# GreptimeTeam/greptimedb

Hardware: AMD Instinct MI355X
Metric: TSBS DevOps ingest rows/sec (whole node) (higher is better)
Workload: dtype f64; 1 GPU; model=tsbs-devops-cpu-only, global_batch=3000, seq_len=0, parallelism=region-shard dp1, scale_per_worker=100, workers=6, pool_rows=2394000, rows_shipped_cross_rank=0, wal=group-commit, no fsync, flush_mb=64, ssts_written=6, device=cuda:0

## Files before the change

csrc/ingest_core.h:

```cpp

#pragma once

#include <cmath>
#include <cstdint>
#include <cstdlib>
#include <cstring>
#include <limits>
#include <string>
#include <utility>
#include <vector>

namespace gdb_ingest {


static inline uint64_t load64(const char* p) {
  uint64_t v;
  std::memcpy(&v, p, 8);
  return v;
}

static inline uint64_t mix64(uint64_t a, uint64_t b) {
  const __uint128_t r = (__uint128_t)a * b;
  return (uint64_t)r ^ (uint64_t)(r >> 64);
}

static inline uint64_t hash64(const char* p, size_t n) {
  const uint64_t K0 = 0x9E3779B97F4A7C15ULL, K1 = 0xA0761D6478BD642FULL,
                 K2 = 0xE7037ED1A0B428DBULL;
  const char* const end = p + n;
  uint64_t s0 = K0 ^ n, s1 = K2;
  size_t left = n;
  while (left >= 32) {
    s0 = mix64(load64(p) ^ K1, load64(p + 8) ^ s0);
// ... 245 lines not shown
  std::vector<std::string> field_names_;
  std::vector<std::pair<size_t, size_t>> fcache_;
  std::vector<uint64_t> stamp_;
  uint64_t stamp_ctr_ = 0;
};


static inline size_t align8(size_t x) { return (x + 7) & ~(size_t)7; }

struct StageLayout {
  size_t ts, fields, dst_off, series, region, total;
  StageLayout(size_t n, size_t nf) {
    ts = 0;
    fields = 8 * n;
    dst_off = fields + 8 * nf * n;
    series = dst_off + 8 * n;
    region = series + align8(4 * n);
    total = region + align8(4 * n);
  }
};

constexpr int kMaxPackedRegions = 16;

enum FusedStatus { FUSED_OK = 0, FUSED_SLOW = 1, FUSED_GROW = 2 };

struct FusedResult {
  FusedStatus status = FUSED_SLOW;
  size_t n = 0;
  size_t need_bytes = 0;
  std::vector<int64_t> counts, mins, maxs;
  std::vector<char> wal;
  std::vector<size_t> wal_off;
  ParseSink sink;
  std::vector<int32_t> own_series;
  std::vector<int64_t> own_ts;
  std::vector<double> own_cols;
};

static inline void fused_ingest(
    LineCore& core, const char* buf, size_t len,
    const int32_t* sid_region, const int32_t* sid_local, size_t lut_len,
    const int64_t* fmap, int nf, size_t n_parser_fields, int n_regions,
    const std::string& hdr_suffix, bool durable, int64_t ts_scale,
    char* stage, size_t stage_bytes, FusedResult& out) {
  const size_t est = LineCore::count_lines(buf, len);
  const size_t F = core.num_fields();
  bool direct = lut_len > 0 && n_regions > 0 && n_regions <= kMaxPackedRegions &&
                n_parser_fields == F && est > 0;
  if (direct) {
    for (int t = 0; t < nf; t++)
      if (fmap[t] >= (int64_t)F) direct = false;
  }
  if (direct) {
    const StageLayout need(est, (size_t)nf);
    if (need.total > stage_bytes) {
      out.status = FUSED_GROW;
      out.need_bytes = need.total;
      return;
    }
  }
  ParseSink& sink = out.sink;
  sink.cap = est;
  sink.col.assign(F, nullptr);
  const StageLayout L(est, (size_t)nf);
  if (direct) {
    sink.ts = reinterpret_cast<int64_t*>(stage + L.ts);
    sink.series = reinterpret_cast<int32_t*>(stage + L.series);
// ... 59 lines not shown
    const int32_t r = sid_region[sid];
    series[i] = sid_local[sid];
    region[i] = r;
    dst_off[i] = cnt[r]++;
    const int64_t t_ns = (int64_t)((uint64_t)ts[i] * (uint64_t)ts_scale);
    int64_t t = t_ns / 1000000;
    if (t_ns % 1000000 < 0) t--;
    ts[i] = t;
    if (t < mn[r]) mn[r] = t;
    if (t > mx[r]) mx[r] = t;
  }
  out.status = FUSED_OK;
  out.wal_off.assign((size_t)n_regions + 1, 0);
  if (!durable) return;

  std::vector<std::string> hdrs(n_regions);
  std::vector<size_t> code_off(n_regions), ts_off(n_regions), f_off(n_regions);
  size_t total = 0;
  for (int r = 0; r < n_regions; r++) {
    out.wal_off[r] = total;
    const size_t m = (size_t)cnt[r];
    if (m == 0) continue;
    hdrs[r] = "{\"n\": " + std::to_string(cnt[r]) + hdr_suffix;
    code_off[r] = total + 4 + hdrs[r].size();
    ts_off[r] = code_off[r] + 4 * m;
    f_off[r] = ts_off[r] + 8 * m;
    total = f_off[r] + 8 * (size_t)nf * m;
  }
  out.wal_off[n_regions] = total;
  out.wal.resize(total);
  char* w = out.wal.data();
  for (int r = 0; r < n_regions; r++) {
    if (cnt[r] == 0) continue;
    const uint32_t hl = (uint32_t)hdrs[r].size();
    std::memcpy(w + out.wal_off[r], &hl, 4);
    std::memcpy(w + out.wal_off[r] + 4, hdrs[r].data(), hl);
  }
  for (size_t i = 0; i < n; i++) {
    const int32_t r = region[i];
    const size_t o = (size_t)dst_off[i];
    const size_t m = (size_t)cnt[r];
    std::memcpy(w + code_off[r] + 4 * o, series + i, 4);
    std::memcpy(w + ts_off[r] + 8 * o, ts + i, 8);
    char* fdst = w + f_off[r];
    for (int t = 0; t < nf; t++)
      std::memcpy(fdst + 8 * ((size_t)t * m + o), fields + (size_t)t * n + i, 8);
  }
}

}
```

csrc/ingest_core_check.cpp:

```cpp

#include <cstdio>
#include <random>
#include <string>
#include <vector>

#include "ingest_core.h"

using namespace gdb_ingest;

static int failures = 0;
#define CHECK(cond)                                                    \
  do {                                                                 \
    if (!(cond)) {                                                     \
      std::printf("CHECK failed %s:%d: %s\n", __FILE__, __LINE__, #cond); \
      failures++;                                                      \
    }                                                                  \
  } while (0)

struct Plain {
  std::vector<int32_t> series;
  std::vector<int64_t> ts;
  std::vector<double> cols;
  ParseSink sink;
  size_t n = 0, cap = 0;
// ... 139 lines not shown
    const int64_t* ts = reinterpret_cast<const int64_t*>(stage.data() + L.ts);
    const double* f = reinterpret_cast<const double*>(stage.data() + L.fields);
    const int64_t* dst = reinterpret_cast<const int64_t*>(stage.data() + L.dst_off);
    const int32_t* se = reinterpret_cast<const int32_t*>(stage.data() + L.series);
    const int32_t* rg = reinterpret_cast<const int32_t*>(stage.data() + L.region);
    std::vector<int64_t> cnt(R, 0);
    for (size_t i = 0; i < n; i++) {
      const int32_t sid = p.series[i];
      CHECK(rg[i] == sid % R && se[i] == sid / R);
      CHECK(dst[i] == cnt[rg[i]]);
      cnt[rg[i]]++;
      CHECK(ts[i] == floor_ms(p.ts[i], scale));
      for (int t = 0; t < nf; t++) {
        const double want = fmap[t] < 0 ? std::nan("") : p.sink.col[fmap[t]][i];
        CHECK(same_double(f[(size_t)t * n + i], want));
      }
    }
    size_t wal = 0;
    for (int r = 0; r < R; r++) {
      CHECK(res.counts[r] == cnt[r]);
      const size_t len = res.wal_off[r + 1] - res.wal_off[r];
      if (cnt[r] == 0) { CHECK(len == 0); continue; }
      uint32_t hl;
      std::memcpy(&hl, res.wal.data() + res.wal_off[r], 4);
      CHECK(len == 4 + hl + (size_t)cnt[r] * (12 + 8 * nf));
      wal += len;
    }
    CHECK(wal == res.wal.size());
  }

  {
    FusedResult res;
    const std::string d = "cpu,hostname=brand_new usage_user=1 5\n";
    fused_ingest(core, d.data(), d.size(), sid_region.data(), sid_local.data(),
                 sid_region.size(), fmap.data(), nf, 4, R, suffix, true, 1,
                 stage.data(), stage.size(), res);
    CHECK(res.status == FUSED_SLOW && res.n == 1 && res.sink.new_tagsets.size() == 1);
    CHECK(res.sink.col[0][0] == 1.0 && std::isnan(res.sink.col[1][0]));
  }
  {
    FusedResult res;
    const std::string d = "cpu,hostname=host_1,region=eu-1,rack=7 usage_user=1,fresh=2 5\n";
    fused_ingest(core, d.data(), d.size(), sid_region.data(), sid_local.data(),
                 sid_region.size(), fmap.data(), nf, 4, R, suffix, true, 1,
                 stage.data(), stage.size(), res);
    CHECK(res.status == FUSED_SLOW && res.n == 1 && core.num_fields() == 5);
    CHECK(res.sink.col.size() == 5 && res.sink.col[4][0] == 2.0);
  }
// ... 27 lines not shown
```

csrc/native.cpp:

```cpp

#include <pybind11/pybind11.h>
#include <pybind11/numpy.h>
#include <pybind11/stl.h>

#include <cerrno>
#include <cmath>
#include <cstdint>
#include <cstring>
#include <fcntl.h>
#include <stdexcept>
#include <string>
#include <unistd.h>
#include <unordered_map>
#include <vector>

#include "ingest_core.h"

namespace py = pybind11;

static uint32_t crc_table[8][256];
static bool crc_init_done = [] {
  for (uint32_t i = 0; i < 256; i++) {
    uint32_t c = i;
    for (int k = 0; k < 8; k++) c = (c & 1) ? 0xEDB88320u ^ (c >> 1) : c >> 1;
    crc_table[0][i] = c;
  }
  for (int t = 1; t < 8; t++)
    for (uint32_t i = 0; i < 256; i++)
      crc_table[t][i] = crc_table[0][crc_table[t - 1][i] & 0xFF] ^
                        (crc_table[t - 1][i] >> 8);
  return true;
}();

static uint32_t crc32_update(uint32_t crc, const uint8_t* buf, size_t len) {
  crc = ~crc;
  while (len >= 8) {
    uint32_t lo, hi;
    std::memcpy(&lo, buf, 4);
    std::memcpy(&hi, buf + 4, 4);
    lo ^= crc;
    crc = crc_table[7][lo & 0xFF] ^ crc_table[6][(lo >> 8) & 0xFF] ^
          crc_table[5][(lo >> 16) & 0xFF] ^ crc_table[4][lo >> 24] ^
          crc_table[3][hi & 0xFF] ^ crc_table[2][(hi >> 8) & 0xFF] ^
          crc_table[1][(hi >> 16) & 0xFF] ^ crc_table[0][hi >> 24];
    buf += 8;
    len -= 8;
  }
  for (size_t i = 0; i < len; i++)
    crc = crc_table[0][(crc ^ buf[i]) & 0xFF] ^ (crc >> 8);
  return ~crc;
}

static inline uint64_t fnv1a(const char* p, size_t n) {
  uint64_t h = 1469598103934665603ULL;
  for (size_t i = 0; i < n; i++) { h ^= (uint8_t)p[i]; h *= 1099511628211ULL; }
  return h;
}


static py::capsule owner_of(void* p) {
  return py::capsule(p, [](void* q) { std::free(q); });
}

class LineParser {
 public:
  py::tuple parse(py::bytes data) {
    char* buf;
    Py_ssize_t len;
    if (PyBytes_AsStringAndSize(data.ptr(), &buf, &len) != 0)
      throw std::runtime_error("expected bytes");
    gdb_ingest::ParseSink sink;
    const size_t F0 = core_.num_fields();
    size_t nrows = 0, est = 0;
    int32_t* series = nullptr;
// ... 7 lines not shown
      block = static_cast<double*>(std::malloc(8 * est * F0 + 8));
      if (series && ts && block) {
        sink.series = series;
        sink.ts = ts;
        sink.cap = est;
        sink.col.resize(F0);
        for (size_t c = 0; c < F0; c++) sink.col[c] = block + c * est;
        nrows = core_.parse(buf, (size_t)len, sink);
      }
    }
    py::capsule so = owner_of(series), to = owner_of(ts), bo = owner_of(block);
    if (!series || !ts || !block) throw std::bad_alloc();
    return make_parse_tuple(
        py::array_t<int32_t>({(py::ssize_t)nrows}, {4}, series, so),
        py::array_t<int64_t>({(py::ssize_t)nrows}, {8}, ts, to),
        sink, nrows, F0, bo);
  }

  py::tuple ingest_batch(
      py::bytes data, py::array_t<int32_t, py::array::c_style> sid_region,
      py::array_t<int32_t, py::array::c_style> sid_local,
      py::array_t<int64_t, py::array::c_style> fmap, size_t n_parser_fields,
      int n_regions, py::bytes hdr_suffix, bool durable, int64_t ts_scale,
      py::array_t<uint8_t, py::array::c_style> stage) {
    char* buf;
    Py_ssize_t len;
    if (PyBytes_AsStringAndSize(data.ptr(), &buf, &len) != 0)
      throw std::runtime_error("expected bytes");
    if (sid_region.ndim() != 1 || sid_local.ndim() != 1 || fmap.ndim() != 1 ||
        stage.ndim() != 1 || sid_local.shape(0) != sid_region.shape(0))
      throw std::runtime_error("ingest_batch: bad argument shapes");
    char* sp = reinterpret_cast<char*>(stage.mutable_data());
    if (reinterpret_cast<uintptr_t>(sp) % 8 != 0)
      throw std::runtime_error("ingest_batch: stage must be 8-byte aligned");
    const std::string suffix = hdr_suffix;
    const size_t F0 = core_.num_fields();
    auto* res = new gdb_ingest::FusedResult();
    py::capsule keep(res, [](void* q) {
      delete static_cast<gdb_ingest::FusedResult*>(q);
    });
    {
      py::gil_scoped_release rel;
      gdb_ingest::fused_ingest(
          core_, buf, (size_t)len, sid_region.data(), sid_local.data(),
          (size_t)sid_region.shape(0), fmap.data(), (int)fmap.shape(0),
          n_parser_fields, n_regions, suffix, durable, ts_scale, sp,
          (size_t)stage.shape(0), *res);
    }
    if (res->status == gdb_ingest::FUSED_GROW)
      return py::make_tuple(2, res->need_bytes);
    if (res->status == gdb_ingest::FUSED_SLOW) {
      const size_t n = res->n;
      py::array_t<int32_t> series((py::ssize_t)n);
      py::array_t<int64_t> ts((py::ssize_t)n);
      if (n) {
        std::memcpy(series.mutable_data(), res->sink.series, 4 * n);
        std::memcpy(ts.mutable_data(), res->sink.ts, 8 * n);
      }
      double* block = static_cast<double*>(std::malloc(8 * n * F0 + 8));
      py::capsule bo = owner_of(block);
      if (!block) throw std::bad_alloc();
      for (size_t c = 0; c < F0 && n; c++)
        std::memcpy(block + c * n, res->sink.col[c], 8 * n);
      for (size_t c = 0; c < F0; c++) res->sink.col[c] = block + c * n;
      return py::make_tuple(1, make_parse_tuple(
          std::move(series), std::move(ts), res->sink, n, F0, bo));
    }
    py::array_t<int64_t> counts(n_regions), mins(n_regions), maxs(n_regions);
    py::list payloads;
    if (res->n) {
      std::memcpy(counts.mutable_data(), res->counts.data(), 8 * (size_t)n_regions);
      std::memcpy(mins.mutable_data(), res->mins.data(), 8 * (size_t)n_regions);
      std::memcpy(maxs.mutable_data(), res->maxs.data(), 8 * (size_t)n_regions);
      for (int r = 0; r < n_regions; r++) {
        const size_t lo = res->wal_off[r], hi = res->wal_off[r + 1];
        if (hi == lo) {
          payloads.append(py::none());
        } else {
          payloads.append(py::array_t<uint8_t>(
              {(py::ssize_t)(hi - lo)}, {1},
              reinterpret_cast<const uint8_t*>(res->wal.data() + lo), keep));
        }
      }
    }
    return py::make_tuple(0, res->n, std::move(counts), std::move(mins),
                          std::move(maxs), std::move(payloads));
  }

  size_t num_series() const { return core_.num_series(); }
  std::vector<std::string> field_names() const { return core_.field_names(); }
  size_t num_fields() const { return core_.num_fields(); }
  size_t intern_capacity() const { return core_.intern_capacity(); }

  py::bytes tagset_str(int32_t sid) const {
    const std::string* s = core_.tagset_str(sid);
    if (!s) throw std::out_of_range("unknown series ref");
    return py::bytes(*s);
  }

  void register_tagset(const std::string& s, int32_t id) { core_.register_tagset(s, id); }
  void register_field(const std::string& name) { core_.register_field(name); }

 private:
  py::tuple make_parse_tuple(py::array_t<int32_t> series, py::array_t<int64_t> ts,
// ... 45 lines not shown
  void close_segment() {
    if (fd_ >= 0) { ::close(fd_); fd_ = -1; }
  }

  void append(uint64_t region_id, uint64_t seq, py::object payload) {
    char* pbuf; Py_ssize_t plen;
    Py_buffer view;
    bool have_view = false;
    if (PyBytes_Check(payload.ptr())) {
      if (PyBytes_AsStringAndSize(payload.ptr(), &pbuf, &plen) != 0)
        throw std::runtime_error("payload must be bytes");
    } else {
      if (PyObject_GetBuffer(payload.ptr(), &view, PyBUF_SIMPLE) != 0)
        throw py::error_already_set();
      have_view = true;
      pbuf = static_cast<char*>(view.buf);
      plen = view.len;
    }
    struct Release {
      Py_buffer* v;
      ~Release() { if (v) PyBuffer_Release(v); }
    } release{have_view ? &view : nullptr};
    py::gil_scoped_release rel;
    uint32_t body_len = 16 + static_cast<uint32_t>(plen);
    size_t off = buf_.size();
    buf_.resize(off + 8 + body_len);
    uint8_t* w = buf_.data() + off;
    std::memcpy(w, &body_len, 4);
    uint8_t hdr[16];
    std::memcpy(hdr, &region_id, 8);
    std::memcpy(hdr + 8, &seq, 8);
    uint32_t crc = crc32_update(0, hdr, 16);
    crc = crc32_update(crc, reinterpret_cast<uint8_t*>(pbuf), plen);
    std::memcpy(w + 4, &crc, 4);
    std::memcpy(w + 8, hdr, 16);
    std::memcpy(w + 24, pbuf, plen);
  }

  uint64_t commit(bool sync) {
    if (fd_ < 0) throw std::runtime_error("wal: no open segment");
    size_t n = buf_.size();
    if (n) {
      py::gil_scoped_release rel;
      const uint8_t* p = buf_.data();
      size_t left = n;
      while (left) {
        ssize_t w = ::write(fd_, p, left);
        if (w < 0) {
          if (errno == EINTR) continue;
          throw std::runtime_error(std::string("wal write failed: ") + strerror(errno));
        }
        p += w; left -= w;
      }
      if (sync && ::fdatasync(fd_) != 0)
        throw std::runtime_error(std::string("wal fdatasync failed: ") + strerror(errno));
    }
    buf_.clear();
    seg_bytes_ += n;
    return seg_bytes_;
  }

  uint64_t segment_bytes() const { return seg_bytes_; }

 private:
  int fd_ = -1;
  std::string path_;
  uint64_t seg_bytes_ = 0;
  std::vector<uint8_t> buf_;
};

static py::list wal_read_segment(const std::string& path) {
  py::list out;
  int fd = ::open(path.c_str(), O_RDONLY);
  if (fd < 0) throw std::runtime_error("wal open failed: " + path);
  off_t sz = ::lseek(fd, 0, SEEK_END);
  ::lseek(fd, 0, SEEK_SET);
  std::vector<uint8_t> data(sz);
  size_t got = 0;
  while (got < static_cast<size_t>(sz)) {
    ssize_t r = ::read(fd, data.data() + got, sz - got);
    if (r <= 0) break;
    got += r;
  }
  ::close(fd);
  size_t off = 0;
  while (off + 8 <= got) {
    uint32_t body_len, crc;
    std::memcpy(&body_len, data.data() + off, 4);
    std::memcpy(&crc, data.data() + off + 4, 4);
    if (body_len < 16 || off + 8 + body_len > got) break;
    const uint8_t* body = data.data() + off + 8;
    if (crc32_update(0, body, body_len) != crc) break;
// ... 968 lines not shown
      std::memcpy(p + ts_off[r] + 8 * o, tp + i, 8);
      char* fdst = p + f_off[r];
      for (int f = 0; f < nf; f++) {
        std::memcpy(fdst + 8 * ((int64_t)f * m + o), fp + (int64_t)f * n + i, 8);
      }
    }
  }
  return py::make_tuple(payloads, std::move(out_mat), std::move(dst_off),
                        std::move(counts), std::move(mins), std::move(maxs));
}

void register_pagedec(py::module_& m);

PYBIND11_MODULE(_native, m) {
  register_pagedec(m);
  m.doc() = "greptimedb_amd host-native ingest path (line parser + WAL)";
  py::class_<LineParser>(m, "LineParser")
      .def(py::init<>())
      .def("parse", &LineParser::parse)
      .def("ingest_batch", &LineParser::ingest_batch, py::arg("data"),
           py::arg("sid_region"), py::arg("sid_local"), py::arg("fmap"),
           py::arg("n_parser_fields"), py::arg("n_regions"),
           py::arg("hdr_suffix"), py::arg("durable"), py::arg("ts_scale"),
           py::arg("stage"))
      .def("num_fields", &LineParser::num_fields)
      .def("intern_capacity", &LineParser::intern_capacity)
      .def("num_series", &LineParser::num_series)
      .def("tagset_str", &LineParser::tagset_str)
      .def("field_names", &LineParser::field_names)
      .def("register_tagset", &LineParser::register_tagset)
      .def("register_field", &LineParser::register_field);
  py::class_<WalWriter>(m, "WalWriter")
      .def(py::init<>())
      .def("open_segment", &WalWriter::open_segment)
      .def("close_segment", &WalWriter::close_segment)
      .def("append", &WalWriter::append)
      .def("commit", &WalWriter::commit, py::arg("sync") = true)
      .def("segment_bytes", &WalWriter::segment_bytes);
  m.def("wal_read_segment", &wal_read_segment);
  m.def("snappy_uncompress", &py_snappy_uncompress);
  m.def("pack_str_col", &pack_str_col);
  m.def("route_ingest", &route_ingest, "K16 host-side ingest router");
  py::class_<PromWriteParser>(m, "PromWriteParser")
      .def(py::init<>())
      .def("parse", &PromWriteParser::parse, py::arg("data"), py::arg("is_snappy") = true)
      .def("num_series", &PromWriteParser::num_series);
  py::class_<OtlpMetricsParser>(m, "OtlpMetricsParser")
      .def(py::init<>())
      .def("parse", &OtlpMetricsParser::parse);
  py::class_<OtlpLogsParser>(m, "OtlpLogsParser")
      .def(py::init<>())
      .def("parse", &OtlpLogsParser::parse);
  py::class_<OtlpTraceParser>(m, "OtlpTraceParser")
      .def(py::init<>())
      .def("parse", &OtlpTraceParser::parse)
      .def("num_series", &OtlpTraceParser::num_series);
  py::class_<Tokenizer>(m, "Tokenizer")
      .def(py::init<>())
      .def("tokenize", &Tokenizer::tokenize)
      .def("term_id", &Tokenizer::term_id)
      .def("intern", &Tokenizer::intern)
      .def("intern_blob", &Tokenizer::intern_blob)
// ... 4 lines not shown
```

greptimedb_amd/engine/engine.py:

```python

from __future__ import annotations

import json
import os
import queue
import threading
from dataclasses import dataclass, field

import numpy as np

from greptimedb_amd.engine.region import Region
from greptimedb_amd.engine.wal import Wal, decode_batch, encode_batch
from greptimedb_amd.models.schema import TableSchema, region_id as make_region_id
from greptimedb_amd.utils.errors import TableAlreadyExists, TableNotFound


@dataclass
class EngineConfig:
    data_dir: str = "./greptime_data"
    device: str = "cpu"
    flush_bytes: int = 512 << 20
    wal_sync: bool = False
    wal_segment_bytes: int = 256 << 20
    wal_shards: int = 1
# ... 313 lines not shown
                mem.max_ts = mx if mem.max_ts is None else max(mem.max_ts, mx)
                region.last_seq = max(region.last_seq, seqs[k])
                region.row_seq += m
        finally:
            for r in reversed(ordered):
                r.lock.release()
        if self.mirror_listeners and n:
            fnames = table.regions[0].field_names
            for k, region in enumerate(regions):
                if int(counts[k]) == 0:
                    continue
                rows = np.flatnonzero(region_of == k)
                for cb in self.mirror_listeners:
                    cb(table, region, series_codes[rows], ts_ms[rows],
                       fields[:, rows], fnames)
        if self.write_listeners and n:
            lo, hi = int(np.min(ts_ms)), int(np.max(ts_ms))
            for cb in self.write_listeners:
                cb(table.schema.name, lo, hi, n)
        return True

    def write_regions_fused(self, table: TableState, slot, n: int, nf: int,
                            counts, mins, maxs, payloads: list,
                            durable: bool = True) -> None:
        import torch
        from greptimedb_amd.ops import cpu_ref
        from greptimedb_amd.ops import kernels as ops

        regions: list[Region] = table.regions
        counts = [int(c) for c in counts]
        seqs = [0] * len(regions)
        if durable:
            for k, p in enumerate(payloads):
                if p is not None:
                    seqs[k] = self.wal.append(regions[k].region_id, p)
        ordered = sorted(regions, key=lambda r: r.region_id)
        for r in ordered:
            r.lock.acquire()
        try:
            bases = []
            for k, region in enumerate(regions):
                mem = region.memtable
                if mem.nf < nf:
                    mem.add_fields(nf - mem.nf)
                need = mem.len + counts[k]
                if need > mem.cap:
                    mem._grow(need)
                bases.append(mem.len)
            dst_ts = [r.memtable.ts for r in regions]
            dst_se = [r.memtable.series for r in regions]
            dst_f = [r.memtable.fields for r in regions]
            if slot.dev is not None:
                ops.scatter_append_packed(slot.host, slot.dev, n, nf, bases,
                                          dst_ts, dst_se, dst_f)
                if slot.event is not None:
# ... 242 lines not shown
```

greptimedb_amd/engine/ingest.py:

```python

from __future__ import annotations

import weakref

import numpy as np

from greptimedb_amd import _native
from greptimedb_amd.engine.engine import MitoEngine, TableState
from greptimedb_amd.engine.series import tsid_hash
from greptimedb_amd.models.schema import ColumnSchema, DataType, SemanticType, TableSchema


def parse_tagset(key: bytes) -> tuple[str, list[tuple[str, str]]]:
    parts = key.decode().split(",")
    measurement = parts[0]
    tags = []
    for p in parts[1:]:
        if "=" in p:
            k, v = p.split("=", 1)
            tags.append((k, v))
    return measurement, tags


STAGE_RING = 3
# ... 18 lines not shown
                slot.event.synchronize()
            except Exception:
                pass
            slot.busy = False


class Ingestor:
    def __init__(self, engine: MitoEngine, default_regions: int | None = None,
                 append_mode: bool = True, durable: bool = True,
                 rank: int = 0, world: int = 1, exchange=None):
        self.engine = engine
        self.parser = _native.LineParser()
        self.append_mode = append_mode
        self.durable = durable
        self.default_regions = default_regions or engine.config.default_regions
        self.rank = rank
        self.world = world
        self.exchange = exchange
        self._remote_cache: dict[bytes, tuple[int, int]] = {}
        self._remote_lock = __import__("threading").Lock()
        self._bulk = engine.config.device.startswith("cuda")
        self._fused = True
        self._packed = True
        self._ring: list[_StageSlot] = []
        self._ring_pos = 0
        self._fused_st = None
        self._fused_lut = None
        weakref.finalize(self, _drain_ring, self._ring)
        self._cap = 1024
        self.sid_region = np.full(self._cap, -1, dtype=np.int32)
        self.sid_local = np.full(self._cap, -1, dtype=np.int32)
        self.sid_rank = np.full(self._cap, -1, dtype=np.int32)
        self.sid_key = np.empty(self._cap, dtype=object)
        self.flat_regions: list = []
        self._region_key: dict = {}
        self._table_field_map: dict = {}
        self._wal_suffix_cache: dict = {}
        self._flat_ridx_cache = None
        self._flat_ridx_table = None
        self.rows_ingested = 0
        self.rows_shipped = 0

    def _flat_region(self, st: TableState, region_idx: int) -> int:
        key = (st.schema.name, region_idx)
        idx = self._region_key.get(key)
        if idx is None:
# ... 160 lines not shown
        st0 = self._fused_st
        if st0 is None or self.engine.tables.get(st0.schema.name) is not st0:
            return self.parser.parse(data)
        regions = st0.regions
        cached = self._table_field_map.get(st0.schema.name)
        nparse = self.parser.num_fields()
        if cached is None or cached[1] != nparse or \
                len(cached[0]) != len(regions[0].field_names) or \
                len(regions) > MAX_PACKED_REGIONS or \
                any(r.text_cols or r.memtable.str_cols or not r.writable
                    for r in regions):
            return self.parser.parse(data)
        lut = self._fused_lut or self._build_fused_lut(st0)
        fmap = cached[0]
        nf = len(fmap)
        suffix = self._wal_suffix(st0)
        if not self._ring:
            self._grow_ring(1 << 16)
        res = None
        for _attempt in range(2):
            slot = self._next_slot()
            res = self.parser.ingest_batch(
                data, lut[0], lut[1], fmap, nparse, len(regions), suffix,
                self.durable, int(ts_scale_to_ns), slot.np)
            if res[0] != 2:
                break
            self._grow_ring(int(res[1]))
        if res[0] == 2:
            raise RuntimeError("ingest stage block still too small after growing")
        if res[0] == 1:
            return res[1]
        _, n, counts, mins, maxs, payloads = res
        if n == 0:
            return 0
        engine = self.engine
        engine.write_regions_fused(st0, slot, n, nf, counts, mins, maxs,
                                   payloads, durable=self.durable)
        slot.busy = slot.event is not None
        self._ring_pos = (self._ring_pos + 1) % len(self._ring)
        if self.durable:
            engine.commit_wal()
        engine.maybe_flush()
        self.rows_ingested += n
        return n

    def ingest_lines(self, data: bytes, ts_scale_to_ns: int = 1) -> int:
        if self._bulk and self._fused:
            got = self._ingest_fused(data, ts_scale_to_ns)
            if isinstance(got, int):
                return got
            series, ts_ns, fields, new_tagsets = got
        else:
            series, ts_ns, fields, new_tagsets = self.parser.parse(data)
        n = len(series)
        if n == 0:
            return 0
        self._check_epoch()
        for sid, key in new_tagsets:
            self._register_tagset(sid, key)
        rank_of = self.sid_rank[series]
# ... 215 lines not shown
```

greptimedb_amd/engine/wal.py:

```python

from __future__ import annotations

import heapq
import json
import os
import re
import struct
import threading

import numpy as np

from greptimedb_amd import _native


def encode_batch(series: np.ndarray, ts_ms: np.ndarray, fields: np.ndarray,
                 field_names: list[str], new_series: list[tuple[int, bytes]],
                 str_cols: dict[str, list] | None = None) -> bytes:
    str_cols = str_cols or {}
    bin_cols = [name for name, vals in str_cols.items()
                if any(isinstance(v, (bytes, bytearray)) for v in vals)]
    hdr = json.dumps({
        "n": int(len(ts_ms)),
        "fields": field_names,
        "strs": list(str_cols),
# ... 84 lines not shown
        for f in os.listdir(self.dir):
            m = _SEG_RE.match(f)
            if not m:
                continue
            if shard is not None and int(m.group(2) or 0) != shard:
                continue
            out.append(f)
        return sorted(out)

    def _shard_of(self, region_id: int) -> _Shard:
        return self.shards[region_id % len(self.shards)]

    def append(self, region_id: int, payload: bytes) -> int:
        with self._lock:
            seq = self.next_seq
            self.next_seq += 1
            self.region_last[region_id] = seq
        sh = self._shard_of(region_id)
        with sh.lock:
            sh.writer.append(region_id, seq, payload)
            sh.dirty = True
        return seq

    def commit(self):
        for sh in self.shards:
            if not sh.dirty:
                continue
            with sh.lock:
                if not sh.dirty:
                    continue
                size = sh.writer.commit(self.sync_on_commit)
                sh.dirty = False
                if size >= self.segment_bytes:
                    sh.writer.close_segment()
                    sh.writer.open_segment(sh.seg_path(self.next_seq))

    def replay(self):
        def shard_stream(shard_idx):
            for seg in self.segments(shard_idx):
                for region, seq, payload in _native.wal_read_segment(
                        os.path.join(self.dir, seg)):
                    yield seq, seg, region, payload

        streams = [shard_stream(i) for i in range(len(self.shards))]
        present = {int(_SEG_RE.match(f).group(2) or 0) for f in self.segments()}
        for extra in sorted(present - set(range(len(self.shards)))):
# ... 24 lines not shown
```

Baseline: 13.60 million rows/s.

## Prebuild WAL frames in fused ingest and use CLMUL CRC32 with crc combine

The fused ingest path now reserves a frame header in front of each region's WAL payload and, when framing is on, computes the payload CRC right after staging. The WAL writer then fills in only the header, folding a 16-byte header CRC into the precomputed payload CRC with crc32_combine. This drops one CRC pass over the payload inside the writer. CRC32 also gains a PCLMUL folding path with a table fallback, the writer buffer moves to a realloc-grown raw buffer instead of a zero-filling vector resize, and sequence numbers are handed out once per batch under a single lock. The cost is a new framed-payload API spanning C++, pybind and Python, with CRC correctness that depends on the combine and CLMUL constants.

```diff
diff --git a/csrc/crc32_fast.h b/csrc/crc32_fast.h
--- /dev/null
+++ b/csrc/crc32_fast.h
@@ -0,0 +1,159 @@
+
+#pragma once
+
+#include <cstddef>
+#include <cstdint>
+#include <cstring>
+
+#if defined(__x86_64__) && (defined(__GNUC__) || defined(__clang__))
+#define GDB_CRC32_HAVE_CLMUL 1
+#include <immintrin.h>
+#else
+#define GDB_CRC32_HAVE_CLMUL 0
+#endif
+
+namespace gdb_crc {
+
+constexpr uint32_t kPoly = 0xEDB88320u;
+
+struct Tables {
+  uint32_t t[8][256];
+  uint32_t x2n[32];
+  Tables() {
+    for (uint32_t i = 0; i < 256; i++) {
+      uint32_t c = i;
+      for (int k = 0; k < 8; k++) c = (c & 1) ? kPoly ^ (c >> 1) : c >> 1;
+      t[0][i] = c;
+    }
+    for (int s = 1; s < 8; s++)
+      for (uint32_t i = 0; i < 256; i++)
+        t[s][i] = t[0][t[s - 1][i] & 0xFF] ^ (t[s - 1][i] >> 8);
+    uint32_t p = 1u << 30;
+    x2n[0] = p;
+    for (int k = 1; k < 32; k++) x2n[k] = p = mulmod(p, p);
+  }
+  static uint32_t mulmod(uint32_t a, uint32_t b) {
+    uint32_t p = 0;
+    for (uint32_t m = 1u << 31; m; m >>= 1) {
+      if (a & m) p ^= b;
+      b = (b & 1) ? (b >> 1) ^ kPoly : b >> 1;
+    }
+    return p;
+  }
+};
+
+inline const Tables& tables() {
+  static const Tables tb;
+  return tb;
+}
+
+static inline uint32_t raw_table(uint32_t crc, const uint8_t* buf, size_t len) {
+  const Tables& tb = tables();
+  while (len >= 8) {
+    uint32_t lo, hi;
+    std::memcpy(&lo, buf, 4);
+    std::memcpy(&hi, buf + 4, 4);
+    lo ^= crc;
+    crc = tb.t[7][lo & 0xFF] ^ tb.t[6][(lo >> 8) & 0xFF] ^
+          tb.t[5][(lo >> 16) & 0xFF] ^ tb.t[4][lo >> 24] ^
+          tb.t[3][hi & 0xFF] ^ tb.t[2][(hi >> 8) & 0xFF] ^
+          tb.t[1][(hi >> 16) & 0xFF] ^ tb.t[0][hi >> 24];
+    buf += 8;
+    len -= 8;
+  }
+  for (size_t i = 0; i < len; i++)
+    crc = tb.t[0][(crc ^ buf[i]) & 0xFF] ^ (crc >> 8);
+  return crc;
+}
+
+static inline uint32_t crc32_table(uint32_t crc, const uint8_t* buf, size_t len) {
+  return ~raw_table(~crc, buf, len);
+}
+
+#if GDB_CRC32_HAVE_CLMUL
+
+static inline bool have_clmul() {
+  static const bool ok = __builtin_cpu_supports("pclmul") &&
+                         __builtin_cpu_supports("sse4.1");
+  return ok;
+}
+
+__attribute__((target("pclmul,sse4.1")))
+static inline uint32_t raw_clmul(uint32_t crc, const uint8_t* buf, size_t len) {
+  const __m128i k1k2 = _mm_set_epi64x(0x01c6e41596, 0x0154442bd4);
+  const __m128i k3k4 = _mm_set_epi64x(0x00ccaa009e, 0x01751997d0);
+  const __m128i* p = reinterpret_cast<const __m128i*>(buf);
+  __m128i x0 = _mm_xor_si128(_mm_loadu_si128(p), _mm_cvtsi32_si128((int)crc));
+  __m128i x1 = _mm_loadu_si128(p + 1);
+  __m128i x2 = _mm_loadu_si128(p + 2);
+  __m128i x3 = _mm_loadu_si128(p + 3);
+  p += 4;
+  len -= 64;
+  while (len >= 64) {
+    const __m128i a0 = _mm_clmulepi64_si128(x0, k1k2, 0x00);
+    const __m128i a1 = _mm_clmulepi64_si128(x1, k1k2, 0x00);
+    const __m128i a2 = _mm_clmulepi64_si128(x2, k1k2, 0x00);
+    const __m128i a3 = _mm_clmulepi64_si128(x3, k1k2, 0x00);
+    x0 = _mm_clmulepi64_si128(x0, k1k2, 0x11);
+    x1 = _mm_clmulepi64_si128(x1, k1k2, 0x11);
+    x2 = _mm_clmulepi64_si128(x2, k1k2, 0x11);
+    x3 = _mm_clmulepi64_si128(x3, k1k2, 0x11);
+    x0 = _mm_xor_si128(_mm_xor_si128(x0, a0), _mm_loadu_si128(p));
+    x1 = _mm_xor_si128(_mm_xor_si128(x1, a1), _mm_loadu_si128(p + 1));
+    x2 = _mm_xor_si128(_mm_xor_si128(x2, a2), _mm_loadu_si128(p + 2));
+    x3 = _mm_xor_si128(_mm_xor_si128(x3, a3), _mm_loadu_si128(p + 3));
+    p += 4;
+    len -= 64;
+  }
+  const __m128i lanes[3] = {x1, x2, x3};
+  for (int i = 0; i < 3; i++) {
+    const __m128i a = _mm_clmulepi64_si128(x0, k3k4, 0x00);
+    x0 = _mm_clmulepi64_si128(x0, k3k4, 0x11);
+    x0 = _mm_xor_si128(_mm_xor_si128(x0, a), lanes[i]);
+  }
+  while (len >= 16) {
+    const __m128i a = _mm_clmulepi64_si128(x0, k3k4, 0x00);
+    x0 = _mm_clmulepi64_si128(x0, k3k4, 0x11);
+    x0 = _mm_xor_si128(_mm_xor_si128(x0, a), _mm_loadu_si128(p));
+    p += 1;
+    len -= 16;
+  }
+  uint8_t tail[16];
+  _mm_storeu_si128(reinterpret_cast<__m128i*>(tail), x0);
+  return raw_table(0, tail, 16);
+}
+
+static inline uint32_t crc32_clmul(uint32_t crc, const uint8_t* buf, size_t len) {
+  crc = ~crc;
+  if (len >= 64) {
+    const size_t body = len & ~(size_t)15;
+    crc = raw_clmul(crc, buf, body);
+    buf += body;
+    len -= body;
+  }
+  return ~raw_table(crc, buf, len);
+}
+
+#else
+
+static inline bool have_clmul() { return false; }
+
+#endif
+
+static inline uint32_t crc32_update(uint32_t crc, const uint8_t* buf, size_t len) {
+#if GDB_CRC32_HAVE_CLMUL
+  if (have_clmul()) return crc32_clmul(crc, buf, len);
+#endif
+  return crc32_table(crc, buf, len);
+}
+
+static inline uint32_t crc32_combine(uint32_t crc_a, uint32_t crc_b, uint64_t len_b) {
+  const Tables& tb = tables();
+  uint32_t p = 1u << 31;
+  unsigned k = 3;
+  for (uint64_t n = len_b; n; n >>= 1, k++)
+    if (n & 1) p = Tables::mulmod(tb.x2n[k & 31], p);
+  return Tables::mulmod(p, crc_a) ^ crc_b;
+}
+
+}
diff --git a/csrc/ingest_core.h b/csrc/ingest_core.h
--- a/csrc/ingest_core.h
+++ b/csrc/ingest_core.h
@@ -6,9 +6,12 @@
 #include <cstdlib>
 #include <cstring>
 #include <limits>
+#include <new>
 #include <string>
 #include <utility>
 #include <vector>
+
+#include "crc32_fast.h"
 
 namespace gdb_ingest {
 
@@ -300,6 +303,71 @@
 
 constexpr int kMaxPackedRegions = 16;
 
+constexpr size_t kWalFrameHeader = 24;
+
+static inline void wal_frame_header(uint8_t* frame, uint64_t region_id,
+                                    uint64_t seq, size_t plen,
+                                    uint32_t payload_crc) {
+  const uint32_t body_len = 16 + (uint32_t)plen;
+  std::memcpy(frame + 8, &region_id, 8);
+  std::memcpy(frame + 16, &seq, 8);
+  const uint32_t crc = gdb_crc::crc32_combine(
+      gdb_crc::crc32_update(0, frame + 8, 16), payload_crc, plen);
+  std::memcpy(frame, &body_len, 4);
+  std::memcpy(frame + 4, &crc, 4);
+}
+
+class WalBuffer {
+ public:
+  WalBuffer() = default;
+  ~WalBuffer() { std::free(buf_); }
+  WalBuffer(const WalBuffer&) = delete;
+  WalBuffer& operator=(const WalBuffer&) = delete;
+
+  void append(uint64_t region_id, uint64_t seq, const uint8_t* payload,
+              size_t plen) {
+    uint8_t* w = grow(kWalFrameHeader + plen);
+    const uint32_t body_len = 16 + (uint32_t)plen;
+    std::memcpy(w, &body_len, 4);
+    std::memcpy(w + 8, &region_id, 8);
+    std::memcpy(w + 16, &seq, 8);
+    uint32_t crc = gdb_crc::crc32_update(0, w + 8, 16);
+    crc = gdb_crc::crc32_update(crc, payload, plen);
+    std::memcpy(w + 4, &crc, 4);
+    if (plen) std::memcpy(w + kWalFrameHeader, payload, plen);
+  }
+
+  void append_framed(uint64_t region_id, uint64_t seq, const uint8_t* frame,
+                     size_t flen, uint32_t payload_crc) {
+    const size_t plen = flen - kWalFrameHeader;
+    uint8_t* w = grow(flen);
+    if (plen) std::memcpy(w + kWalFrameHeader, frame + kWalFrameHeader, plen);
+    wal_frame_header(w, region_id, seq, plen, payload_crc);
+  }
+
+  const uint8_t* data() const { return buf_; }
+  size_t size() const { return size_; }
+  size_t capacity() const { return cap_; }
+  void clear() { size_ = 0; }
+
+ private:
+  uint8_t* grow(size_t add) {
+    if (add > cap_ - size_) {
+      size_t cap = cap_ ? cap_ : (size_t)1 << 16;
+      while (cap - size_ < add) cap *= 2;
+      uint8_t* nb = static_cast<uint8_t*>(std::realloc(buf_, cap));
+      if (!nb) throw std::bad_alloc();
+      buf_ = nb;
+      cap_ = cap;
+    }
+    uint8_t* w = buf_ + size_;
+    size_ += add;
+    return w;
+  }
+  uint8_t* buf_ = nullptr;
+  size_t size_ = 0, cap_ = 0;
+};
+
 enum FusedStatus { FUSED_OK = 0, FUSED_SLOW = 1, FUSED_GROW = 2 };
 
 struct FusedResult {
@@ -309,6 +377,7 @@
   std::vector<int64_t> counts, mins, maxs;
   std::vector<char> wal;
   std::vector<size_t> wal_off;
+  std::vector<uint32_t> wal_crc;
   ParseSink sink;
   std::vector<int32_t> own_series;
   std::vector<int64_t> own_ts;
@@ -320,7 +389,7 @@
     const int32_t* sid_region, const int32_t* sid_local, size_t lut_len,
     const int64_t* fmap, int nf, size_t n_parser_fields, int n_regions,
     const std::string& hdr_suffix, bool durable, int64_t ts_scale,
-    char* stage, size_t stage_bytes, FusedResult& out) {
+    char* stage, size_t stage_bytes, FusedResult& out, bool checksum = false) {
   const size_t est = LineCore::count_lines(buf, len);
   const size_t F = core.num_fields();
   bool direct = lut_len > 0 && n_regions > 0 && n_regions <= kMaxPackedRegions &&
@@ -426,7 +495,7 @@
     const size_t m = (size_t)cnt[r];
     if (m == 0) continue;
     hdrs[r] = "{\"n\": " + std::to_string(cnt[r]) + hdr_suffix;
-    code_off[r] = total + 4 + hdrs[r].size();
+    code_off[r] = total + kWalFrameHeader + 4 + hdrs[r].size();
     ts_off[r] = code_off[r] + 4 * m;
     f_off[r] = ts_off[r] + 8 * m;
     total = f_off[r] + 8 * (size_t)nf * m;
@@ -437,8 +506,9 @@
   for (int r = 0; r < n_regions; r++) {
     if (cnt[r] == 0) continue;
     const uint32_t hl = (uint32_t)hdrs[r].size();
-    std::memcpy(w + out.wal_off[r], &hl, 4);
-    std::memcpy(w + out.wal_off[r] + 4, hdrs[r].data(), hl);
+    char* payload = w + out.wal_off[r] + kWalFrameHeader;
+    std::memcpy(payload, &hl, 4);
+    std::memcpy(payload + 4, hdrs[r].data(), hl);
   }
   for (size_t i = 0; i < n; i++) {
     const int32_t r = region[i];
@@ -450,6 +520,14 @@
     for (int t = 0; t < nf; t++)
       std::memcpy(fdst + 8 * ((size_t)t * m + o), fields + (size_t)t * n + i, 8);
   }
-}
-
-}
+  if (!checksum) return;
+  out.wal_crc.assign(n_regions, 0);
+  for (int r = 0; r < n_regions; r++) {
+    if (cnt[r] == 0) continue;
+    const size_t lo = out.wal_off[r] + kWalFrameHeader;
+    out.wal_crc[r] = gdb_crc::crc32_update(
+        0, reinterpret_cast<const uint8_t*>(w + lo), out.wal_off[r + 1] - lo);
+  }
+}
+
+}
diff --git a/csrc/ingest_core_check.cpp b/csrc/ingest_core_check.cpp
--- a/csrc/ingest_core_check.cpp
+++ b/csrc/ingest_core_check.cpp
@@ -185,8 +185,8 @@
       const size_t len = res.wal_off[r + 1] - res.wal_off[r];
       if (cnt[r] == 0) { CHECK(len == 0); continue; }
       uint32_t hl;
-      std::memcpy(&hl, res.wal.data() + res.wal_off[r], 4);
-      CHECK(len == 4 + hl + (size_t)cnt[r] * (12 + 8 * nf));
+      std::memcpy(&hl, res.wal.data() + res.wal_off[r] + kWalFrameHeader, 4);
+      CHECK(len == kWalFrameHeader + 4 + hl + (size_t)cnt[r] * (12 + 8 * nf));
       wal += len;
     }
     CHECK(wal == res.wal.size());
diff --git a/csrc/native.cpp b/csrc/native.cpp
--- a/csrc/native.cpp
+++ b/csrc/native.cpp
@@ -14,42 +14,12 @@
 #include <unordered_map>
 #include <vector>
 
+#include "crc32_fast.h"
 #include "ingest_core.h"
 
 namespace py = pybind11;
 
-static uint32_t crc_table[8][256];
-static bool crc_init_done = [] {
-  for (uint32_t i = 0; i < 256; i++) {
-    uint32_t c = i;
-    for (int k = 0; k < 8; k++) c = (c & 1) ? 0xEDB88320u ^ (c >> 1) : c >> 1;
-    crc_table[0][i] = c;
-  }
-  for (int t = 1; t < 8; t++)
-    for (uint32_t i = 0; i < 256; i++)
-      crc_table[t][i] = crc_table[0][crc_table[t - 1][i] & 0xFF] ^
-                        (crc_table[t - 1][i] >> 8);
-  return true;
-}();
-
-static uint32_t crc32_update(uint32_t crc, const uint8_t* buf, size_t len) {
-  crc = ~crc;
-  while (len >= 8) {
-    uint32_t lo, hi;
-    std::memcpy(&lo, buf, 4);
-    std::memcpy(&hi, buf + 4, 4);
-    lo ^= crc;
-    crc = crc_table[7][lo & 0xFF] ^ crc_table[6][(lo >> 8) & 0xFF] ^
-          crc_table[5][(lo >> 16) & 0xFF] ^ crc_table[4][lo >> 24] ^
-          crc_table[3][hi & 0xFF] ^ crc_table[2][(hi >> 8) & 0xFF] ^
-          crc_table[1][(hi >> 16) & 0xFF] ^ crc_table[0][hi >> 24];
-    buf += 8;
-    len -= 8;
-  }
-  for (size_t i = 0; i < len; i++)
-    crc = crc_table[0][(crc ^ buf[i]) & 0xFF] ^ (crc >> 8);
-  return ~crc;
-}
+using gdb_crc::crc32_update;
 
 static inline uint64_t fnv1a(const char* p, size_t n) {
   uint64_t h = 1469598103934665603ULL;
@@ -103,7 +73,7 @@
       py::array_t<int32_t, py::array::c_style> sid_local,
       py::array_t<int64_t, py::array::c_style> fmap, size_t n_parser_fields,
       int n_regions, py::bytes hdr_suffix, bool durable, int64_t ts_scale,
-      py::array_t<uint8_t, py::array::c_style> stage) {
+      py::array_t<uint8_t, py::array::c_style> stage, bool framed) {
     char* buf;
     Py_ssize_t len;
     if (PyBytes_AsStringAndSize(data.ptr(), &buf, &len) != 0)
@@ -126,7 +96,7 @@
           core_, buf, (size_t)len, sid_region.data(), sid_local.data(),
           (size_t)sid_region.shape(0), fmap.data(), (int)fmap.shape(0),
           n_parser_fields, n_regions, suffix, durable, ts_scale, sp,
-          (size_t)stage.shape(0), *res);
+          (size_t)stage.shape(0), *res, framed);
     }
     if (res->status == gdb_ingest::FUSED_GROW)
       return py::make_tuple(2, res->need_bytes);
@@ -154,13 +124,20 @@
       std::memcpy(mins.mutable_data(), res->mins.data(), 8 * (size_t)n_regions);
       std::memcpy(maxs.mutable_data(), res->maxs.data(), 8 * (size_t)n_regions);
       for (int r = 0; r < n_regions; r++) {
-        const size_t lo = res->wal_off[r], hi = res->wal_off[r + 1];
+        size_t lo = res->wal_off[r];
+        const size_t hi = res->wal_off[r + 1];
         if (hi == lo) {
           payloads.append(py::none());
+          continue;
+        }
+        if (!framed) lo += gdb_ingest::kWalFrameHeader;
+        py::array_t<uint8_t> view(
+            {(py::ssize_t)(hi - lo)}, {1},
+            reinterpret_cast<const uint8_t*>(res->wal.data() + lo), keep);
+        if (framed) {
+          payloads.append(py::make_tuple(std::move(view), res->wal_crc[r]));
         } else {
-          payloads.append(py::array_t<uint8_t>(
-              {(py::ssize_t)(hi - lo)}, {1},
-              reinterpret_cast<const uint8_t*>(res->wal.data() + lo), keep));
+          payloads.append(std::move(view));
         }
       }
     }
@@ -252,19 +229,24 @@
       ~Release() { if (v) PyBuffer_Release(v); }
     } release{have_view ? &view : nullptr};
     py::gil_scoped_release rel;
-    uint32_t body_len = 16 + static_cast<uint32_t>(plen);
-    size_t off = buf_.size();
-    buf_.resize(off + 8 + body_len);
-    uint8_t* w = buf_.data() + off;
-    std::memcpy(w, &body_len, 4);
-    uint8_t hdr[16];
-    std::memcpy(hdr, &region_id, 8);
-    std::memcpy(hdr + 8, &seq, 8);
-    uint32_t crc = crc32_update(0, hdr, 16);
-    crc = crc32_update(crc, reinterpret_cast<uint8_t*>(pbuf), plen);
-    std::memcpy(w + 4, &crc, 4);
-    std::memcpy(w + 8, hdr, 16);
-    std::memcpy(w + 24, pbuf, plen);
+    buf_.append(region_id, seq, reinterpret_cast<const uint8_t*>(pbuf), (size_t)plen);
+  }
+
+  void append_framed(uint64_t region_id, uint64_t seq, py::buffer frame,
+                     uint32_t payload_crc) {
+    Py_buffer view;
+    if (PyObject_GetBuffer(frame.ptr(), &view, PyBUF_SIMPLE) != 0)
+      throw py::error_already_set();
+    struct Release {
+      Py_buffer* v;
+      ~Release() { PyBuffer_Release(v); }
+    } release{&view};
+    constexpr size_t H = gdb_ingest::kWalFrameHeader;
+    if ((size_t)view.len < H || (size_t)view.len - H > UINT32_MAX - 16)
+      throw std::runtime_error("append_framed: bad frame length");
+    py::gil_scoped_release rel;
+    buf_.append_framed(region_id, seq, static_cast<const uint8_t*>(view.buf),
+                       (size_t)view.len, payload_crc);
   }
 
   uint64_t commit(bool sync) {
@@ -296,8 +278,25 @@
   int fd_ = -1;
   std::string path_;
   uint64_t seg_bytes_ = 0;
-  std::vector<uint8_t> buf_;
+  gdb_ingest::WalBuffer buf_;
 };
+
+static uint32_t py_crc32(py::buffer data, const std::string& impl, uint32_t start) {
+  py::buffer_info info = data.request();
+  if (info.ndim > 1 || (info.ndim == 1 && info.strides[0] != info.itemsize))
+    throw std::runtime_error("crc32: need a contiguous buffer");
+  const uint8_t* p = static_cast<const uint8_t*>(info.ptr);
+  const size_t len = (size_t)info.size * (size_t)info.itemsize;
+  if (impl == "auto") return gdb_crc::crc32_update(start, p, len);
+  if (impl == "table") return gdb_crc::crc32_table(start, p, len);
+  if (impl == "clmul") {
+#if GDB_CRC32_HAVE_CLMUL
+    if (gdb_crc::have_clmul()) return gdb_crc::crc32_clmul(start, p, len);
+#endif
+    throw std::runtime_error("crc32: clmul is not available on this CPU");
+  }
+  throw std::invalid_argument("crc32: impl must be auto, table or clmul");
+}
 
 static py::list wal_read_segment(const std::string& path) {
   py::list out;
@@ -1312,7 +1311,7 @@
            py::arg("sid_region"), py::arg("sid_local"), py::arg("fmap"),
            py::arg("n_parser_fields"), py::arg("n_regions"),
            py::arg("hdr_suffix"), py::arg("durable"), py::arg("ts_scale"),
-           py::arg("stage"))
+           py::arg("stage"), py::arg("framed") = false)
       .def("num_fields", &LineParser::num_fields)
       .def("intern_capacity", &LineParser::intern_capacity)
       .def("num_series", &LineParser::num_series)
@@ -1325,9 +1324,16 @@
       .def("open_segment", &WalWriter::open_segment)
       .def("close_segment", &WalWriter::close_segment)
       .def("append", &WalWriter::append)
+      .def("append_framed", &WalWriter::append_framed, py::arg("region_id"),
+           py::arg("seq"), py::arg("frame"), py::arg("payload_crc"))
       .def("commit", &WalWriter::commit, py::arg("sync") = true)
       .def("segment_bytes", &WalWriter::segment_bytes);
   m.def("wal_read_segment", &wal_read_segment);
+  m.def("crc32", &py_crc32, py::arg("data"), py::arg("impl") = "auto",
+        py::arg("start") = 0);
+  m.def("crc32_combine", &gdb_crc::crc32_combine, py::arg("crc_a"),
+        py::arg("crc_b"), py::arg("len_b"));
+  m.def("crc32_has_clmul", &gdb_crc::have_clmul);
   m.def("snappy_uncompress", &py_snappy_uncompress);
   m.def("pack_str_col", &pack_str_col);
   m.def("route_ingest", &route_ingest, "K16 host-side ingest router");
diff --git a/csrc/wal_frame_check.cpp b/csrc/wal_frame_check.cpp
--- /dev/null
+++ b/csrc/wal_frame_check.cpp
@@ -0,0 +1,186 @@
+
+#include <cstdio>
+#include <random>
+#include <string>
+#include <vector>
+
+#include "crc32_fast.h"
+#include "ingest_core.h"
+
+using namespace gdb_ingest;
+
+static int failures = 0;
+#define CHECK(cond)                                                    \
+  do {                                                                 \
+    if (!(cond)) {                                                     \
+      std::printf("CHECK failed %s:%d: %s\n", __FILE__, __LINE__, #cond); \
+      failures++;                                                      \
+    }                                                                  \
+  } while (0)
+
+static uint32_t crc_ref(uint32_t crc, const uint8_t* p, size_t n) {
+  crc = ~crc;
+  for (size_t i = 0; i < n; i++) {
+    crc ^= p[i];
+    for (int k = 0; k < 8; k++) crc = (crc & 1) ? (crc >> 1) ^ 0xEDB88320u : crc >> 1;
+  }
+  return ~crc;
+}
+
+static const size_t kLens[] = {0, 1, 7, 8, 9, 15, 16, 17, 63, 64, 65, 127, 128,
+                               129, 255, 256, 257, 4099};
+
+static void crc_cases() {
+  CHECK(gdb_crc::crc32_update(0, reinterpret_cast<const uint8_t*>("123456789"), 9) ==
+        0xCBF43926u);
+  std::mt19937_64 rng(7);
+  for (size_t len : kLens) {
+    for (size_t off = 0; off < 8; off++) {
+      std::vector<uint8_t> buf(off + len);
+      for (auto& b : buf) b = (uint8_t)rng();
+      const uint8_t* p = buf.data() + off;
+      const uint32_t start = (uint32_t)rng() | 1u;
+      const uint32_t want = crc_ref(start, p, len);
+      CHECK(gdb_crc::crc32_table(start, p, len) == want);
+      CHECK(gdb_crc::crc32_update(start, p, len) == want);
+#if GDB_CRC32_HAVE_CLMUL
+      if (gdb_crc::have_clmul()) CHECK(gdb_crc::crc32_clmul(start, p, len) == want);
+#endif
+    }
+  }
+  for (size_t la : {(size_t)0, (size_t)16, (size_t)1001}) {
+    for (size_t lb : kLens) {
+      std::vector<uint8_t> ab(la + lb);
+      for (auto& b : ab) b = (uint8_t)rng();
+      const uint32_t ca = crc_ref(0, ab.data(), la);
+      const uint32_t cb = crc_ref(0, ab.data() + la, lb);
+      CHECK(gdb_crc::crc32_combine(ca, cb, lb) == crc_ref(0, ab.data(), la + lb));
+    }
+  }
+}
+
+static void buffer_cases() {
+  std::mt19937_64 rng(11);
+  WalBuffer plain, framed;
+  for (int i = 0; i < 200; i++) {
+    size_t plen = rng() % 5001;
+    if (i % 67 == 66) plen = 300000 + rng() % 1000;
+    std::vector<uint8_t> frame(kWalFrameHeader + plen);
+    for (auto& b : frame) b = (uint8_t)rng();
+    const uint8_t* payload = frame.data() + kWalFrameHeader;
+    const uint64_t region = rng(), seq = rng();
+    plain.append(region, seq, payload, plen);
+    framed.append_framed(region, seq, frame.data(), frame.size(),
+                         gdb_crc::crc32_update(0, payload, plen));
+    CHECK(plain.size() == framed.size());
+    if (i == 120) {
+      CHECK(std::memcmp(plain.data(), framed.data(), plain.size()) == 0);
+      plain.clear();
+      framed.clear();
+    }
+  }
+  CHECK(plain.size() == framed.size() && plain.size() <= plain.capacity());
+  CHECK(std::memcmp(plain.data(), framed.data(), plain.size()) == 0);
+  size_t off = 0, frames = 0;
+  while (off + 8 <= framed.size()) {
+    uint32_t body_len, crc;
+    std::memcpy(&body_len, framed.data() + off, 4);
+    std::memcpy(&crc, framed.data() + off + 4, 4);
+    CHECK(body_len >= 16 && off + 8 + body_len <= framed.size());
+    if (body_len < 16 || off + 8 + body_len > framed.size()) break;
+    CHECK(crc_ref(0, framed.data() + off + 8, body_len) == crc);
+    off += 8 + body_len;
+    frames++;
+  }
+  CHECK(off == framed.size() && frames == 79);
+}
+
+static void fused_cases() {
+  std::mt19937_64 rng(13);
+  LineCore core;
+  const int n_hosts = 37, R = 4;
+  std::string warm;
+  for (int h = 0; h < n_hosts; h++)
+    warm += "cpu,hostname=host_" + std::to_string(h) + " a=1,b=2,c=3i 1\n";
+  {
+    ParseSink sink;
+    std::vector<int32_t> se(n_hosts);
+    std::vector<int64_t> ts(n_hosts);
+    sink.series = se.data();
+    sink.ts = ts.data();
+    sink.cap = n_hosts;
+    CHECK(core.parse(warm.data(), warm.size(), sink) == (size_t)n_hosts);
+  }
+  std::vector<int32_t> sid_region(n_hosts), sid_local(n_hosts);
+  for (int s = 0; s < n_hosts; s++) { sid_region[s] = s % 3; sid_local[s] = s / 3; }
+  const std::vector<int64_t> fmap = {1, -1, 0, 2};
+  const int nf = (int)fmap.size();
+  const std::string suffix = ", \"fields\": [\"b\", \"x\", \"a\", \"c\"]}";
+  for (int rows : {1, 2, 7, 50, 333}) {
+    std::string data;
+    for (int i = 0; i < rows; i++)
+      data += "cpu,hostname=host_" + std::to_string(rng() % n_hosts) + " a=" +
+              std::to_string((int)(rng() % 1000)) + ".5,b=" + std::to_string(i) +
+              ",c=" + std::to_string(rng() % 99) + "i " +
+              std::to_string(1000000 * (int64_t)(rng() % 100000)) + "\n";
+    const StageLayout L((size_t)rows, (size_t)nf);
+    std::vector<char> stage(L.total);
+    FusedResult res;
+    fused_ingest(core, data.data(), data.size(), sid_region.data(), sid_local.data(),
+                 sid_region.size(), fmap.data(), nf, 3, R, suffix, true, 1,
+                 stage.data(), stage.size(), res, true);
+    CHECK(res.status == FUSED_OK && res.n == (size_t)rows);
+    if (res.status != FUSED_OK) continue;
+    CHECK(res.wal_off.size() == (size_t)R + 1 && res.wal_crc.size() == (size_t)R);
+    CHECK(res.wal_off[R] == res.wal.size());
+    WalBuffer plain, framed;
+    for (int r = 0; r < R; r++) {
+      const size_t lo = res.wal_off[r], hi = res.wal_off[r + 1];
+      if (res.counts[r] == 0) { CHECK(hi == lo); continue; }
+      CHECK(hi - lo > kWalFrameHeader);
+      const uint8_t* frame = reinterpret_cast<const uint8_t*>(res.wal.data() + lo);
+      const uint8_t* payload = frame + kWalFrameHeader;
+      const size_t plen = hi - lo - kWalFrameHeader;
+      uint32_t hl;
+      std::memcpy(&hl, payload, 4);
+      CHECK(plen == 4 + hl + (size_t)res.counts[r] * (12 + 8 * nf));
+      CHECK(res.wal_crc[r] == crc_ref(0, payload, plen));
+      plain.append(100 + r, 1000 + r, payload, plen);
+      framed.append_framed(100 + r, 1000 + r, frame, hi - lo, res.wal_crc[r]);
+    }
+    CHECK(res.counts[3] == 0);
+    CHECK(plain.size() == framed.size() &&
+          std::memcmp(plain.data(), framed.data(), plain.size()) == 0);
+
+    std::vector<char> stage2(L.total);
+    FusedResult nocrc, nolog;
+    fused_ingest(core, data.data(), data.size(), sid_region.data(), sid_local.data(),
+                 sid_region.size(), fmap.data(), nf, 3, R, suffix, true, 1,
+                 stage2.data(), stage2.size(), nocrc);
+    CHECK(nocrc.status == FUSED_OK && nocrc.wal_crc.empty());
+    CHECK(nocrc.wal_off == res.wal_off);
+    for (int r = 0; r < R; r++) {
+      if (res.counts[r] == 0) continue;
+      const size_t lo = res.wal_off[r] + kWalFrameHeader;
+      CHECK(std::memcmp(nocrc.wal.data() + lo, res.wal.data() + lo,
+                        res.wal_off[r + 1] - lo) == 0);
+    }
+    fused_ingest(core, data.data(), data.size(), sid_region.data(), sid_local.data(),
+                 sid_region.size(), fmap.data(), nf, 3, R, suffix, false, 1,
+                 stage2.data(), stage2.size(), nolog, true);
+    CHECK(nolog.status == FUSED_OK && nolog.wal.empty() && nolog.wal_crc.empty());
+  }
+}
+
+int main() {
+  crc_cases();
+  buffer_cases();
+  fused_cases();
+  if (failures) {
+    std::printf("wal_frame_check: %d failure(s)\n", failures);
+    return 1;
+  }
+  std::printf("wal_frame_check ok (clmul %s)\n",
+              gdb_crc::have_clmul() ? "checked" : "not available");
+  return 0;
+}
diff --git a/greptimedb_amd/engine/engine.py b/greptimedb_amd/engine/engine.py
--- a/greptimedb_amd/engine/engine.py
+++ b/greptimedb_amd/engine/engine.py
@@ -359,7 +359,7 @@
 
     def write_regions_fused(self, table: TableState, slot, n: int, nf: int,
                             counts, mins, maxs, payloads: list,
-                            durable: bool = True) -> None:
+                            durable: bool = True, framed: bool = False) -> None:
         import torch
         from greptimedb_amd.ops import cpu_ref
         from greptimedb_amd.ops import kernels as ops
@@ -367,7 +367,13 @@
         regions: list[Region] = table.regions
         counts = [int(c) for c in counts]
         seqs = [0] * len(regions)
-        if durable:
+        if durable and framed:
+            live = [k for k, p in enumerate(payloads) if p is not None]
+            got = self.wal.append_frames(
+                [(regions[k].region_id, *payloads[k]) for k in live])
+            for k, seq in zip(live, got):
+                seqs[k] = seq
+        elif durable:
             for k, p in enumerate(payloads):
                 if p is not None:
                     seqs[k] = self.wal.append(regions[k].region_id, p)
diff --git a/greptimedb_amd/engine/ingest.py b/greptimedb_amd/engine/ingest.py
--- a/greptimedb_amd/engine/ingest.py
+++ b/greptimedb_amd/engine/ingest.py
@@ -64,6 +64,7 @@
         self._bulk = engine.config.device.startswith("cuda")
         self._fused = True
         self._packed = True
+        self._framed = True
         self._ring: list[_StageSlot] = []
         self._ring_pos = 0
         self._fused_st = None
@@ -270,7 +271,7 @@
             slot = self._next_slot()
             res = self.parser.ingest_batch(
                 data, lut[0], lut[1], fmap, nparse, len(regions), suffix,
-                self.durable, int(ts_scale_to_ns), slot.np)
+                self.durable, int(ts_scale_to_ns), slot.np, self._framed)
             if res[0] != 2:
                 break
             self._grow_ring(int(res[1]))
@@ -283,7 +284,8 @@
             return 0
         engine = self.engine
         engine.write_regions_fused(st0, slot, n, nf, counts, mins, maxs,
-                                   payloads, durable=self.durable)
+                                   payloads, durable=self.durable,
+                                   framed=self._framed)
         slot.busy = slot.event is not None
         self._ring_pos = (self._ring_pos + 1) % len(self._ring)
         if self.durable:
diff --git a/greptimedb_amd/engine/wal.py b/greptimedb_amd/engine/wal.py
--- a/greptimedb_amd/engine/wal.py
+++ b/greptimedb_amd/engine/wal.py
@@ -130,6 +130,22 @@
             sh.dirty = True
         return seq
 
+    def append_frames(self, entries: list) -> list[int]:
+        n = len(entries)
+        region_last = self.region_last
+        with self._lock:
+            seq0 = self.next_seq
+            self.next_seq = seq0 + n
+            for i, e in enumerate(entries):
+                region_last[e[0]] = seq0 + i
+        nsh = len(self.shards)
+        for i, (region_id, frame, crc) in enumerate(entries):
+            sh = self.shards[region_id % nsh]
+            with sh.lock:
+                sh.writer.append_framed(region_id, seq0 + i, frame, crc)
+                sh.dirty = True
+        return list(range(seq0, seq0 + n))
+
     def commit(self):
         for sh in self.shards:
             if not sh.dirty:
```

Measured after the change: 14.74 million rows/s (median of 5 runs). 1.08x the previous value.
